# SonyCSLParis/vqcpc-bach

Measured on AMD Instinct MI355X. Metric: encoder-train windows/sec (Bach 4-voice, seq=256), higher is better.
Workload: dtype f32

## Files before the change

vqcpc_bach_amd/csrc/gru.hip:

```cpp
#include "common.h"

namespace vq {

__device__ __forceinline__ float sigmoidf_(float x) { return 1.0f / (1.0f + expf(-x)); }

struct GiTok {
    const int64_t* tokens;
    int L, p, voff, vmax;
};

template <bool TOK>
__device__ __forceinline__ const float* gi_row(const float* gi, const GiTok& tk, int64_t b, int H) {
    if constexpr (TOK) {
        const int tok = min(max((int)tk.tokens[b * tk.L + tk.p], 0), tk.vmax - 1);
        return gi + (int64_t)(tk.voff + tok) * 3 * H;
    } else {
        return gi + b * 3 * H;
    }
}

template <bool TOK>
__global__ __launch_bounds__(256) void gru_cell_fwd_kernel(const float* __restrict__ gi, GiTok tk, const float* __restrict__ gh,
                                                           const float* __restrict__ h_prev, float* __restrict__ h_out,
                                                           float* __restrict__ y_out, int64_t B, int H, uint32_t thr,
                                                           float inv_keep, uint64_t seed, uint64_t idx_base) {
    const int64_t e = (int64_t)blockIdx.x * blockDim.x + threadIdx.x;
    if (e >= B * H) return;
    const int64_t b = e / H;
    const int c = (int)(e - b * H);
    const float* gib = gi_row<TOK>(gi, tk, b, H);
    const float* ghb = gh + b * 3 * H;
    const float r = sigmoidf_(gib[c] + ghb[c]);
    const float u = sigmoidf_(gib[H + c] + ghb[H + c]);
    const float n = tanhf(gib[2 * H + c] + r * ghb[2 * H + c]);
    const float hp = h_prev ? h_prev[e] : 0.0f;
    const float h = (1.0f - u) * n + u * hp;
    h_out[e] = h;
    if (y_out) y_out[e] = h * drop_scale(seed, idx_base + (uint64_t)e, thr, inv_keep);
}

template <bool TOK>
__global__ __launch_bounds__(256) void gru_cell_bwd_kernel(const float* __restrict__ gi, GiTok tk, const float* __restrict__ gh,
                                                           const float* __restrict__ h_prev, const float* __restrict__ d_y,
                                                           const float* __restrict__ d_h, float* __restrict__ d_gi,
                                                           float* __restrict__ d_gh, float* __restrict__ d_hprev, int64_t B,
                                                           int H, uint32_t thr, float inv_keep, uint64_t seed,
                                                           uint64_t idx_base) {
    const int64_t e = (int64_t)blockIdx.x * blockDim.x + threadIdx.x;
    if (e >= B * H) return;
    const int64_t b = e / H;
    const int c = (int)(e - b * H);
    const int64_t o = b * 3 * H + c;
    const float* gib = gi_row<TOK>(gi, tk, b, H) + c;
    const float ghn = gh[o + 2 * H];
    const float r = sigmoidf_(gib[0] + gh[o]);
    const float u = sigmoidf_(gib[H] + gh[o + H]);
    const float n = tanhf(gib[2 * H] + r * ghn);
    const float hp = h_prev ? h_prev[e] : 0.0f;
    float dh = d_h ? d_h[e] : 0.0f;
    if (d_y) dh += d_y[e] * drop_scale(seed, idx_base + (uint64_t)e, thr, inv_keep);
    const float da_n = dh * (1.0f - u) * (1.0f - n * n);
    const float da_u = dh * (hp - n) * u * (1.0f - u);
    const float da_r = da_n * ghn * r * (1.0f - r);
    d_gi[o] = da_r;
    d_gi[o + H] = da_u;
    d_gi[o + 2 * H] = da_n;
    d_gh[o] = da_r;
    d_gh[o + H] = da_u;
    d_gh[o + 2 * H] = da_n * r;
    d_hprev[e] = dh * u;
}

typedef float gru_f16 __attribute__((ext_vector_type(16)));
constexpr int kGruNW = 8;

#define GRU_MFMA4(ACC, AV, BV)                                                     \
    ACC = __builtin_amdgcn_mfma_f32_32x32x2f32(AV.x, BV.x, ACC, 0, 0, 0);           \
    ACC = __builtin_amdgcn_mfma_f32_32x32x2f32(AV.y, BV.y, ACC, 0, 0, 0);           \
    ACC = __builtin_amdgcn_mfma_f32_32x32x2f32(AV.z, BV.z, ACC, 0, 0, 0);           \
    ACC = __builtin_amdgcn_mfma_f32_32x32x2f32(AV.w, BV.w, ACC, 0, 0, 0);

template <bool TOK>
__global__ __launch_bounds__(kGruNW * 64) void gru_step_fwd_kernel(const float* __restrict__ gi, GiTok tk, const float* __restrict__ w_hh,
                                                                   const float* __restrict__ b_hh,
                                                                   const float* __restrict__ h_prev, float* __restrict__ gh,
                                                                   float* __restrict__ h_out, float* __restrict__ y_out,
                                                                   int B, int H, uint32_t thr, float inv_keep, uint64_t seed,
                                                                   uint64_t idx_base) {
    extern __shared__ float gru_red[];
    const int lane = threadIdx.x & 63, wave = threadIdx.x >> 6, g = lane >> 5, l31 = lane & 31;
    const int i = blockIdx.y * 32 + l31, j = blockIdx.x * 32 + l31;
    float e_gi[2][3], e_hp[2];
    int e_row[2];
#pragma unroll
    for (int q = 0; q < 2; ++q) {
        const int r = 2 * wave + q;
        e_row[q] = blockIdx.y * 32 + (r & 3) + 8 * (r >> 2) + 4 * g;
        const int rr = min(e_row[q], B - 1);
        const float* gib = gi_row<TOK>(gi, tk, rr, H) + j;
        e_gi[q][0] = gib[0];
        e_gi[q][1] = gib[H];
        e_gi[q][2] = gib[2 * H];
        e_hp[q] = h_prev ? h_prev[(int64_t)rr * H + j] : 0.0f;
    }
    const float br = b_hh[j], bu = b_hh[H + j], bn = b_hh[2 * H + j];
    gru_f16 acc[3];
#pragma unroll
    for (int q = 0; q < 3; ++q)
#pragma unroll
        for (int r = 0; r < 16; ++r) acc[q][r] = 0.0f;
    if (h_prev != nullptr) {
        const int len = H / (2 * kGruNW);
        const int k0 = (wave * 2 + g) * len;
        const float* ap = h_prev + (int64_t)min(i, B - 1) * H + k0;
        const float* bp = w_hh + (int64_t)j * H + k0;
        int kk = 0;
        for (; kk + 16 <= len; kk += 16) {
            float4 a[4], b[3][4];
#pragma unroll
            for (int v = 0; v < 4; ++v) {
                a[v] = *reinterpret_cast<const float4*>(ap + kk + 4 * v);
#pragma unroll
                for (int q = 0; q < 3; ++q) b[q][v] = *reinterpret_cast<const float4*>(bp + (int64_t)q * H * H + kk + 4 * v);
            }
#pragma unroll
            for (int v = 0; v < 4; ++v) {
                GRU_MFMA4(acc[0], a[v], b[0][v])
                GRU_MFMA4(acc[1], a[v], b[1][v])
                GRU_MFMA4(acc[2], a[v], b[2][v])
            }
        }
        for (; kk < len; kk += 4) {
            const float4 a = *reinterpret_cast<const float4*>(ap + kk);
#pragma unroll
            for (int q = 0; q < 3; ++q) {
                const float4 b = *reinterpret_cast<const float4*>(bp + (int64_t)q * H * H + kk);
                GRU_MFMA4(acc[q], a, b)
            }
        }
#pragma unroll
        for (int q = 0; q < 3; ++q)
#pragma unroll
            for (int r = 0; r < 16; ++r) gru_red[((wave * 3 + q) * 16 + r) * 64 + lane] = acc[q][r];
        __syncthreads();
    }
#pragma unroll
    for (int q = 0; q < 2; ++q) {
        const int r = 2 * wave + q;
        float v3[3] = {0.0f, 0.0f, 0.0f};
        if (h_prev != nullptr) {
#pragma unroll
            for (int w = 0; w < kGruNW; ++w)
#pragma unroll
                for (int t = 0; t < 3; ++t) v3[t] += gru_red[((w * 3 + t) * 16 + r) * 64 + lane];
        }
        if (e_row[q] < B) {
            const float vr = v3[0] + br, vu = v3[1] + bu, vn = v3[2] + bn;
            const int64_t o = (int64_t)e_row[q] * 3 * H + j, e = (int64_t)e_row[q] * H + j;
            gh[o] = vr; gh[o + H] = vu; gh[o + 2 * H] = vn;
            const float rr = sigmoidf_(e_gi[q][0] + vr);
            const float uu = sigmoidf_(e_gi[q][1] + vu);
            const float nn = tanhf(e_gi[q][2] + rr * vn);
            const float hv = (1.0f - uu) * nn + uu * e_hp[q];
            h_out[e] = hv;
            if (y_out) y_out[e] = hv * drop_scale(seed, idx_base + (uint64_t)e, thr, inv_keep);
        }
    }
}

template <bool TOK>
__global__ __launch_bounds__(kGruNW * 64) void gru_step_bwd_kernel(const float* __restrict__ dgh_next,
                                                                   const float* __restrict__ whh_t, float* __restrict__ dhp,
                                                                   const float* __restrict__ gi, GiTok tk, const float* __restrict__ gh,
                                                                   const float* __restrict__ h_prev,
                                                                   const float* __restrict__ d_y, float* __restrict__ d_gi,
                                                                   float* __restrict__ d_gh, int B, int H, uint32_t thr,
                                                                   float inv_keep, uint64_t seed, uint64_t idx_base) {
    extern __shared__ float gru_red[];
    const int lane = threadIdx.x & 63, wave = threadIdx.x >> 6, g = lane >> 5, l31 = lane & 31;
    const int i = blockIdx.y * 32 + l31, j = blockIdx.x * 32 + l31;
    const int K3 = 3 * H;
    float e_gi[2][3], e_gh[2][3], e_hp[2], e_dh[2];
    int e_row[2];
#pragma unroll
    for (int q = 0; q < 2; ++q) {
        const int r = 2 * wave + q;
        e_row[q] = blockIdx.y * 32 + (r & 3) + 8 * (r >> 2) + 4 * g;
        const int rr = min(e_row[q], B - 1);
        const int64_t o = (int64_t)rr * 3 * H + j, e = (int64_t)rr * H + j;
        const float* gib = gi_row<TOK>(gi, tk, rr, H) + j;
#pragma unroll
        for (int t = 0; t < 3; ++t) {
            e_gi[q][t] = gib[(int64_t)t * H];
            e_gh[q][t] = gh[o + (int64_t)t * H];
        }
        e_hp[q] = h_prev ? h_prev[e] : 0.0f;
        e_dh[q] = dhp[e];
        if (d_y) e_dh[q] += d_y[e] * drop_scale(seed, idx_base + (uint64_t)e, thr, inv_keep);
    }
    const int len = K3 / (2 * kGruNW);
    const int k0 = (wave * 2 + g) * len;
    const float* ap = dgh_next + (int64_t)min(i, B - 1) * K3 + k0;
    const float* bp = whh_t + (int64_t)j * K3 + k0;
    gru_f16 acc;
#pragma unroll
    for (int r = 0; r < 16; ++r) acc[r] = 0.0f;
    int kk = 0;
    for (; kk + 32 <= len; kk += 32) {
        float4 a[8], b[8];
#pragma unroll
        for (int v = 0; v < 8; ++v) {
            a[v] = *reinterpret_cast<const float4*>(ap + kk + 4 * v);
            b[v] = *reinterpret_cast<const float4*>(bp + kk + 4 * v);
        }
#pragma unroll
        for (int v = 0; v < 8; ++v) { GRU_MFMA4(acc, a[v], b[v]) }
    }
    for (; kk < len; kk += 4) {
        const float4 a = *reinterpret_cast<const float4*>(ap + kk);
        const float4 b = *reinterpret_cast<const float4*>(bp + kk);
        GRU_MFMA4(acc, a, b)
    }
#pragma unroll
    for (int r = 0; r < 16; ++r) gru_red[(wave * 16 + r) * 64 + lane] = acc[r];
    __syncthreads();
#pragma unroll
    for (int q = 0; q < 2; ++q) {
        const int r = 2 * wave + q;
        float dh = 0.0f;
#pragma unroll
        for (int w = 0; w < kGruNW; ++w) dh += gru_red[(w * 16 + r) * 64 + lane];
        if (e_row[q] < B) {
            const int64_t o = (int64_t)e_row[q] * 3 * H + j, e = (int64_t)e_row[q] * H + j;
            dh += e_dh[q];
            const float ghn = e_gh[q][2];
            const float rr = sigmoidf_(e_gi[q][0] + e_gh[q][0]);
            const float uu = sigmoidf_(e_gi[q][1] + e_gh[q][1]);
            const float nn = tanhf(e_gi[q][2] + rr * ghn);
            const float hp = e_hp[q];
            const float da_n = dh * (1.0f - uu) * (1.0f - nn * nn);
            const float da_u = dh * (hp - nn) * uu * (1.0f - uu);
            const float da_r = da_n * ghn * rr * (1.0f - rr);
            d_gi[o] = da_r; d_gi[o + H] = da_u; d_gi[o + 2 * H] = da_n;
            d_gh[o] = da_r; d_gh[o + H] = da_u; d_gh[o + 2 * H] = da_n * rr;
            dhp[e] = dh * uu;
        }
    }
}
#undef GRU_MFMA4

constexpr int kTokSegU = 16;
constexpr int kTokSegChunkRows = 128;
constexpr int kTokSegMaxChunks = 64;

__global__ __launch_bounds__(256) void gru_tok_segsum_kernel(const float* __restrict__ g, const int64_t* __restrict__ tokens,
                                                             float* __restrict__ ws, int64_t R, int rows_per_chunk, int L, int p,
                                                             int vmax, int C) {
    extern __shared__ __attribute__((aligned(16))) float tok_acc[];
    for (int i = threadIdx.x; i < vmax * 256; i += 256) tok_acc[i] = 0.0f;
    __syncthreads();
    const int ctiles = (C + 255) / 256;
    const int ct = blockIdx.x % ctiles, chunk = blockIdx.x / ctiles;
    const int col = ct * 256 + threadIdx.x;
    const bool cok = col < C;
    const int64_t b0 = (int64_t)chunk * rows_per_chunk;
    const int64_t b1 = min(b0 + rows_per_chunk, R);
    const float* gp = g + (cok ? col : 0);
    float* mine = tok_acc + threadIdx.x;
    for (int64_t b = b0; b < b1; b += kTokSegU) {
        float v[kTokSegU];
        const int64_t trow = min(b + (int)(threadIdx.x & 63) % kTokSegU, b1 - 1);
        const int tokv = min(max((int)tokens[trow * L + p], 0), vmax - 1);
#pragma unroll
        for (int u = 0; u < kTokSegU; ++u) {
            const int64_t row = min(b + u, b1 - 1);
            v[u] = b + u < b1 ? gp[row * C] : 0.0f;
        }
#pragma unroll
        for (int u = 0; u < kTokSegU; ++u) mine[__builtin_amdgcn_readlane(tokv, u) * 256] += v[u];
    }
    if (cok) {
        float* dst = ws + (int64_t)chunk * vmax * C;
        for (int t = 0; t < vmax; ++t) dst[(int64_t)t * C + col] = tok_acc[t * 256 + threadIdx.x];
    }
}

static int tok_segsum_chunks(int64_t R) {
    return (int)std::max<int64_t>(1, std::min<int64_t>(kTokSegMaxChunks, ceil_div(R, kTokSegChunkRows)));
}

static int gi_tok_args(const char* who, const int64_t* tokens, int64_t B, int L, int p, int n_voices, int vmax, GiTok* tk) {
    VQ_REQUIRE(tokens && L >= 1 && p >= 0 && p < L && n_voices >= 1 && vmax >= 1 && B < (1 << 30),
               "%s: bad token arguments (L=%d p=%d n_voices=%d vmax=%d)", who, L, p, n_voices, vmax);
    *tk = GiTok{tokens, L, p, (p % n_voices) * vmax, vmax};
    return VQCPC_OK;
}

}

#include <algorithm>
using namespace vq;

template <bool TOK>
static int cell_fwd_launch(const float* gi, GiTok tk, const float* gh, const float* h_prev, float* h_out, float* y_out, int64_t B,
                           int H, float drop_p, uint64_t seed, uint64_t idx_base, void* stream) {
    VQ_REQUIRE(gi && gh && h_out && B >= 0 && H >= 1, "gru_cell_fwd: bad arguments");
    VQ_REQUIRE(drop_p >= 0.f && drop_p < 1.f, "gru_cell_fwd: bad dropout probability");
    hipLaunchKernelGGL(gru_cell_fwd_kernel<TOK>, dim3((unsigned)ceil_div(B * H, 256)), dim3(256), 0, (hipStream_t)stream, gi, tk, gh,
                       h_prev, h_out, y_out, B, H, drop_threshold(drop_p), 1.0f / (1.0f - drop_p), seed, idx_base);
    VQ_CHECK_LAUNCH("gru_cell_fwd");
    return VQCPC_OK;
}

template <bool TOK>
static int cell_bwd_launch(const float* gi, GiTok tk, const float* gh, const float* h_prev, const float* d_y, const float* d_h,
                           float* d_gi, float* d_gh, float* d_hprev, int64_t B, int H, float drop_p, uint64_t seed,
                           uint64_t idx_base, void* stream) {
    VQ_REQUIRE(gi && gh && d_gi && d_gh && d_hprev && (d_y || d_h) && B >= 0 && H >= 1, "gru_cell_bwd: bad arguments");
    VQ_REQUIRE(drop_p >= 0.f && drop_p < 1.f, "gru_cell_bwd: bad dropout probability");
    hipLaunchKernelGGL(gru_cell_bwd_kernel<TOK>, dim3((unsigned)ceil_div(B * H, 256)), dim3(256), 0, (hipStream_t)stream, gi, tk, gh,
                       h_prev, d_y, d_h, d_gi, d_gh, d_hprev, B, H, drop_threshold(drop_p), 1.0f / (1.0f - drop_p), seed,
                       idx_base);
    VQ_CHECK_LAUNCH("gru_cell_bwd");
    return VQCPC_OK;
}

template <bool TOK>
static int step_fwd_launch(const float* gi, GiTok tk, const float* w_hh, const float* b_hh, const float* h_prev, float* gh,
                           float* h_out, float* y_out, int64_t B, int H, float drop_p, uint64_t seed, uint64_t idx_base,
                           void* stream) {
    VQ_REQUIRE(gi && w_hh && b_hh && gh && h_out, "gru_step_fwd: null pointer");
    VQ_REQUIRE(vqcpc_gru_step_supported(B, H) && B < (1 << 30), "gru_step_fwd: needs H %% 64 == 0 (B=%lld H=%d)", (long long)B, H);
    VQ_REQUIRE(drop_p >= 0.f && drop_p < 1.f, "gru_step_fwd: bad dropout probability");
    VQ_REQUIRE(aligned16(w_hh) && (!h_prev || aligned16(h_prev)), "gru_step_fwd: operands must be 16-byte aligned");
    const size_t lds = (size_t)kGruNW * 3 * 16 * 64 * sizeof(float);
    static bool attr = false;
    if (!attr) {
        (void)hipFuncSetAttribute((const void*)gru_step_fwd_kernel<TOK>, hipFuncAttributeMaxDynamicSharedMemorySize, (int)lds);
        attr = true;
    }
    hipLaunchKernelGGL(gru_step_fwd_kernel<TOK>, dim3(H / 32, (unsigned)ceil_div(B, 32)), dim3(kGruNW * 64), lds, (hipStream_t)stream,
                       gi, tk, w_hh, b_hh, h_prev, gh, h_out, y_out, (int)B, H, drop_threshold(drop_p), 1.0f / (1.0f - drop_p), seed,
                       idx_base);
    VQ_CHECK_LAUNCH("gru_step_fwd");
    return VQCPC_OK;
}

template <bool TOK>
static int step_bwd_launch(const float* dgh_next, const float* whh_t, float* dhp, const float* gi, GiTok tk, const float* gh,
                           const float* h_prev, const float* d_y, float* d_gi, float* d_gh, int64_t B, int H, float drop_p,
                           uint64_t seed, uint64_t idx_base, void* stream) {
    VQ_REQUIRE(dgh_next && whh_t && dhp && gi && gh && d_gi && d_gh, "gru_step_bwd: null pointer");
    VQ_REQUIRE(vqcpc_gru_step_supported(B, H) && B < (1 << 30), "gru_step_bwd: needs H %% 64 == 0 (B=%lld H=%d)", (long long)B, H);
    VQ_REQUIRE(drop_p >= 0.f && drop_p < 1.f, "gru_step_bwd: bad dropout probability");
    VQ_REQUIRE(aligned16(dgh_next) && aligned16(whh_t), "gru_step_bwd: operands must be 16-byte aligned");
    const size_t lds = (size_t)kGruNW * 16 * 64 * sizeof(float);
    hipLaunchKernelGGL(gru_step_bwd_kernel<TOK>, dim3(H / 32, (unsigned)ceil_div(B, 32)), dim3(kGruNW * 64), lds, (hipStream_t)stream,
                       dgh_next, whh_t, dhp, gi, tk, gh, h_prev, d_y, d_gi, d_gh, (int)B, H, drop_threshold(drop_p),
                       1.0f / (1.0f - drop_p), seed, idx_base);
    VQ_CHECK_LAUNCH("gru_step_bwd");
    return VQCPC_OK;
}

extern "C" {

int vqcpc_gru_cell_fwd(const float* gi, const float* gh, const float* h_prev, float* h_out, float* y_out, int64_t B, int H,
                       float drop_p, uint64_t seed, uint64_t idx_base, void* stream) {
    if (B == 0) return VQCPC_OK;
    return cell_fwd_launch<false>(gi, GiTok{}, gh, h_prev, h_out, y_out, B, H, drop_p, seed, idx_base, stream);
}

int vqcpc_gru_cell_bwd(const float* gi, const float* gh, const float* h_prev, const float* d_y, const float* d_h, float* d_gi,
                       float* d_gh, float* d_hprev, int64_t B, int H, float drop_p, uint64_t seed, uint64_t idx_base,
                       void* stream) {
    if (B == 0) return VQCPC_OK;
    return cell_bwd_launch<false>(gi, GiTok{}, gh, h_prev, d_y, d_h, d_gi, d_gh, d_hprev, B, H, drop_p, seed, idx_base, stream);
}

int vqcpc_gru_step_supported(int64_t B, int H) { return (B >= 1 && H >= 64 && H % 64 == 0 && H <= 4096) ? 1 : 0; }

int vqcpc_gru_step_fwd(const float* gi, const float* w_hh, const float* b_hh, const float* h_prev, float* gh, float* h_out,
                       float* y_out, int64_t B, int H, float drop_p, uint64_t seed, uint64_t idx_base, void* stream) {
    if (B == 0) return VQCPC_OK;
    return step_fwd_launch<false>(gi, GiTok{}, w_hh, b_hh, h_prev, gh, h_out, y_out, B, H, drop_p, seed, idx_base, stream);
}

int vqcpc_gru_step_bwd(const float* dgh_next, const float* whh_t, float* dhp, const float* gi, const float* gh,
// ... 74 lines not shown
```

vqcpc_bach_amd/csrc/util.hip:

```cpp
#include <stdarg.h>

#include <algorithm>

#include "common.h"

namespace vq {

static thread_local char g_err[512] = "";

void set_error(const char* fmt, ...) {
    va_list ap;
    va_start(ap, fmt);
    vsnprintf(g_err, sizeof(g_err), fmt, ap);
    va_end(ap);
}

constexpr int kRedCols = 64, kRedGroups = 16;

__global__ __launch_bounds__(kRedCols * kRedGroups) void reduce_splits_kernel(const float* __restrict__ ws,
                                                                              int64_t stride, int nsplit,
                                                                              float* __restrict__ out, int64_t count,
                                                                              const float* __restrict__ ws2, int64_t stride2,
                                                                              float* __restrict__ out2, int64_t count2,
                                                                              int accumulate) {
    __shared__ float part[kRedGroups][kRedCols];
    const int tx = threadIdx.x % kRedCols, ty = threadIdx.x / kRedCols;
    int64_t col = (int64_t)blockIdx.x * kRedCols + tx;
    const int64_t first = (count + kRedCols - 1) / kRedCols * kRedCols;
    if (col >= first) {
        col -= first;
        ws = ws2;
        stride = stride2;
        out = out2;
        count = count2;
    }
    float acc = 0.0f;
    if (col < count) {
        int s = ty;
        for (; s + 3 * kRedGroups < nsplit; s += 4 * kRedGroups) {
            const float a = ws[(int64_t)s * stride + col];
            const float b = ws[(int64_t)(s + kRedGroups) * stride + col];
            const float c = ws[(int64_t)(s + 2 * kRedGroups) * stride + col];
            const float d = ws[(int64_t)(s + 3 * kRedGroups) * stride + col];
            acc = ((acc + a) + b) + (c + d);
        }
        for (; s < nsplit; s += kRedGroups) acc += ws[(int64_t)s * stride + col];
    }
    part[ty][tx] = acc;
    __syncthreads();
    if (ty == 0 && col < count) {
        float tot = accumulate ? out[col] : 0.0f;
#pragma unroll
        for (int g = 0; g < kRedGroups; ++g) tot += part[g][tx];
        out[col] = tot;
    }
}

constexpr int kRedVecThreads = 256;

__global__ __launch_bounds__(kRedVecThreads) void reduce_splits_vec_kernel(const float* __restrict__ ws, int64_t stride,
                                                                          int nsplit, float* __restrict__ out, int64_t count,
                                                                          const float* __restrict__ ws2, int64_t stride2,
                                                                          float* __restrict__ out2, int64_t count2,
                                                                          int accumulate) {
    int64_t q = (int64_t)blockIdx.x * kRedVecThreads + threadIdx.x;
    const int64_t first = (count / 4 + kRedVecThreads - 1) / kRedVecThreads * kRedVecThreads;
    if (q >= first) {
        q -= first;
        ws = ws2;
        stride = stride2;
        out = out2;
        count = count2;
    }
    if (q * 4 >= count) return;
    const float4* p = reinterpret_cast<const float4*>(ws) + q;
    const int64_t st4 = stride / 4;
    float4 acc = make_float4(0.f, 0.f, 0.f, 0.f);
#define RV_ADD(X, Y) make_float4(X.x + Y.x, X.y + Y.y, X.z + Y.z, X.w + Y.w)
    int s = 0;
    for (; s + 7 < nsplit; s += 8) {
        const float4 v0 = p[(s + 0) * st4], v1 = p[(s + 1) * st4], v2 = p[(s + 2) * st4], v3 = p[(s + 3) * st4];
        const float4 v4 = p[(s + 4) * st4], v5 = p[(s + 5) * st4], v6 = p[(s + 6) * st4], v7 = p[(s + 7) * st4];
        const float4 a = RV_ADD(v0, v1), b = RV_ADD(v2, v3), c = RV_ADD(v4, v5), d = RV_ADD(v6, v7);
        const float4 ab = RV_ADD(a, b), cd = RV_ADD(c, d);
        const float4 t = RV_ADD(ab, cd);
        acc = RV_ADD(acc, t);
    }
    for (; s < nsplit; ++s) {
        const float4 v = p[s * st4];
        acc = RV_ADD(acc, v);
    }
    float4* o = reinterpret_cast<float4*>(out) + q;
    if (accumulate) {
        const float4 prev = *o;
        acc = RV_ADD(prev, acc);
    }
#undef RV_ADD
    *o = acc;
}

static bool reduce_vec_ok(const float* ws, int64_t stride, const float* out, int64_t count) {
    return count <= 0 || (count % 4 == 0 && stride % 4 == 0 && aligned16(ws) && aligned16(out));
}

int launch_reduce_splits2(const float* ws, int64_t stride, int nsplit, float* out, int64_t count, const float* ws2,
                          int64_t stride2, float* out2, int64_t count2, int accumulate, hipStream_t stream) {
    if (count <= 0 && count2 <= 0) return VQCPC_OK;
    if (count >= (1 << 16) && nsplit <= 64 && reduce_vec_ok(ws, stride, out, count) &&
        reduce_vec_ok(ws2, stride2, out2, count2)) {
        const int64_t blocks = ceil_div(count / 4, (int64_t)kRedVecThreads) +
                               ceil_div(std::max<int64_t>(count2, 0) / 4, (int64_t)kRedVecThreads);
        hipLaunchKernelGGL(reduce_splits_vec_kernel, dim3((unsigned)blocks), dim3(kRedVecThreads), 0, stream, ws, stride,
                           nsplit, out, count, ws2, stride2, out2, std::max<int64_t>(count2, 0), accumulate);
        VQ_CHECK_LAUNCH("reduce_splits_vec");
        return VQCPC_OK;
    }
    const int64_t blocks = ceil_div(std::max<int64_t>(count, 0), kRedCols) + ceil_div(std::max<int64_t>(count2, 0), kRedCols);
    hipLaunchKernelGGL(reduce_splits_kernel, dim3((unsigned)blocks), dim3(kRedCols * kRedGroups), 0, stream, ws, stride,
                       nsplit, out, std::max<int64_t>(count, 0), ws2, stride2, out2, std::max<int64_t>(count2, 0), accumulate);
    VQ_CHECK_LAUNCH("reduce_splits");
    return VQCPC_OK;
}

constexpr int kRedMany = 32;
struct RedManyArgs {
    const float* ws[kRedMany];
    float* out[kRedMany];
    int stride[kRedMany], nsplit[kRedMany], count[kRedMany];
    int blk_begin[kRedMany + 1];
    int n, accumulate;
};

__global__ __launch_bounds__(kRedCols * kRedGroups) void reduce_many_kernel(const RedManyArgs g) {
    __shared__ float part[kRedGroups][kRedCols];
    const int b = (int)blockIdx.x;
    int p = 0;
    for (int i = 1; i < g.n; ++i) p += (b >= g.blk_begin[i]) ? 1 : 0;
    p = __builtin_amdgcn_readfirstlane(p);
    const float* __restrict__ ws = g.ws[p];
    const int64_t stride = g.stride[p];
    const int nsplit = g.nsplit[p], count = g.count[p];
    const int tx = threadIdx.x % kRedCols, ty = threadIdx.x / kRedCols;
    const int col = (b - g.blk_begin[p]) * kRedCols + tx;
    float acc = 0.0f;
    if (col < count) {
        int s = ty;
        for (; s + 3 * kRedGroups < nsplit; s += 4 * kRedGroups) {
            const float a = ws[(int64_t)s * stride + col];
            const float b2 = ws[(int64_t)(s + kRedGroups) * stride + col];
            const float c = ws[(int64_t)(s + 2 * kRedGroups) * stride + col];
            const float d = ws[(int64_t)(s + 3 * kRedGroups) * stride + col];
            acc = ((acc + a) + b2) + (c + d);
        }
        for (; s < nsplit; s += kRedGroups) acc += ws[(int64_t)s * stride + col];
    }
    part[ty][tx] = acc;
    __syncthreads();
    if (ty == 0 && col < count) {
        float* out = g.out[p];
        float tot = g.accumulate ? out[col] : 0.0f;
#pragma unroll
        for (int q = 0; q < kRedGroups; ++q) tot += part[q][tx];
        out[col] = tot;
    }
}

__global__ __launch_bounds__(kRedVecThreads) void reduce_many_vec_kernel(const RedManyArgs g) {
    const int b = (int)blockIdx.x;
    int p = 0;
    for (int i = 1; i < g.n; ++i) p += (b >= g.blk_begin[i]) ? 1 : 0;
    p = __builtin_amdgcn_readfirstlane(p);
    const int64_t q = (int64_t)(b - g.blk_begin[p]) * kRedVecThreads + threadIdx.x;
    if (q * 4 >= g.count[p]) return;
    const float4* ptr = reinterpret_cast<const float4*>(g.ws[p]) + q;
    const int64_t st4 = g.stride[p] / 4;
    const int nsplit = g.nsplit[p];
    float4 acc = make_float4(0.f, 0.f, 0.f, 0.f);
#define RV_ADD(X, Y) make_float4(X.x + Y.x, X.y + Y.y, X.z + Y.z, X.w + Y.w)
    int s = 0;
    for (; s + 7 < nsplit; s += 8) {
        const float4 v0 = ptr[(s + 0) * st4], v1 = ptr[(s + 1) * st4], v2 = ptr[(s + 2) * st4], v3 = ptr[(s + 3) * st4];
        const float4 v4 = ptr[(s + 4) * st4], v5 = ptr[(s + 5) * st4], v6 = ptr[(s + 6) * st4], v7 = ptr[(s + 7) * st4];
        const float4 a = RV_ADD(v0, v1), bb = RV_ADD(v2, v3), c = RV_ADD(v4, v5), d = RV_ADD(v6, v7);
        const float4 ab = RV_ADD(a, bb), cd = RV_ADD(c, d);
        const float4 t = RV_ADD(ab, cd);
        acc = RV_ADD(acc, t);
    }
    for (; s < nsplit; ++s) {
        const float4 v = ptr[s * st4];
        acc = RV_ADD(acc, v);
    }
    float4* o = reinterpret_cast<float4*>(g.out[p]) + q;
    if (g.accumulate) {
        const float4 prev = *o;
        acc = RV_ADD(prev, acc);
    }
#undef RV_ADD
    *o = acc;
}

int launch_reduce_splits(const float* ws, int64_t stride, int nsplit, float* out, int64_t count, int accumulate,
                         hipStream_t stream) {
    return launch_reduce_splits2(ws, stride, nsplit, out, count, nullptr, 0, nullptr, 0, accumulate, stream);
}

__global__ __launch_bounds__(256) void dropout_mask_kernel(float* mask, int64_t n, uint32_t thr, uint64_t seed) {
    int64_t i = (int64_t)blockIdx.x * blockDim.x + threadIdx.x;
    const int64_t step = (int64_t)gridDim.x * blockDim.x;
    for (; i < n; i += step) mask[i] = (thr == 0 || rng_u24(seed, (uint64_t)i) >= thr) ? 1.0f : 0.0f;
}

__global__ __launch_bounds__(256) void transpose_kernel(const float* __restrict__ in, float* __restrict__ out, int R,
                                                        int C) {
    __shared__ float tile[32][33];
    const int tx = threadIdx.x & 31, ty = threadIdx.x >> 5;
    const int c0 = blockIdx.x * 32, r0 = blockIdx.y * 32;
#pragma unroll
    for (int k = 0; k < 4; ++k) {
        int r = r0 + ty + k * 8, c = c0 + tx;
        if (r < R && c < C) tile[ty + k * 8][tx] = in[(int64_t)r * C + c];
    }
    __syncthreads();
#pragma unroll
    for (int k = 0; k < 4; ++k) {
        int c = c0 + ty + k * 8, r = r0 + tx;
        if (r < R && c < C) out[(int64_t)c * R + r] = tile[tx][ty + k * 8];
    }
}

__global__ __launch_bounds__(256) void transpose_many_kernel(const float* __restrict__ base_in, float* __restrict__ base_out,
                                                             const int64_t* __restrict__ desc, int n) {
    __shared__ float tile[32][33];
    int lo = 0, hi = n - 1;
    const int64_t t = blockIdx.x;
    while (lo < hi) {
        const int mid = (lo + hi + 1) >> 1;
        if (desc[4 * mid + 3] <= t) lo = mid; else hi = mid - 1;
    }
    const int64_t off = desc[4 * lo];
    const int R = (int)desc[4 * lo + 1], C = (int)desc[4 * lo + 2];
    const int local = (int)(t - desc[4 * lo + 3]), tiles_c = (C + 31) / 32;
    const float* in = base_in + off;
    float* out = base_out + off;
    const int tx = threadIdx.x & 31, ty = threadIdx.x >> 5;
    const int c0 = (local % tiles_c) * 32, r0 = (local / tiles_c) * 32;
#pragma unroll
    for (int k = 0; k < 4; ++k) {
        const int r = r0 + ty + k * 8, c = c0 + tx;
        if (r < R && c < C) tile[ty + k * 8][tx] = in[(int64_t)r * C + c];
    }
    __syncthreads();
#pragma unroll
    for (int k = 0; k < 4; ++k) {
        const int c = c0 + ty + k * 8, r = r0 + tx;
        if (r < R && c < C) out[(int64_t)c * R + r] = tile[tx][ty + k * 8];
    }
}

__device__ __forceinline__ float selu_f(float h, float s) {
    const double alpha = 1.6732632423543772848170429916717, scale = 1.0507009873554804934193349852946;
    const double x = (double)h * (double)s;
    return (float)(scale * (x > 0.0 ? x : alpha * expm1(x)));
}
__device__ __forceinline__ float selu_grad(float x) {
    const float alpha = 1.6732632423543772848170429916717f, scale = 1.0507009873554804934193349852946f;
    return scale * (x > 0.0f ? 1.0f : alpha * __expf(x));
}

__global__ __launch_bounds__(256) void dropout_selu_fwd_kernel(const float* __restrict__ h, float* __restrict__ out,
                                                               int64_t n, uint32_t thr, float inv_keep, uint64_t seed) {
    int64_t i = (int64_t)blockIdx.x * blockDim.x + threadIdx.x;
    const int64_t step = (int64_t)gridDim.x * blockDim.x;
// ... 69 lines not shown
        v[i] = vi;
        g[i] = gi;
        p[i] -= lr_over_bc1 * (mi / (sqrtf(vi) * inv_sqrt_bc2 + eps));
    }
}


static SaltAddrFn g_salt_fns[32];
static int g_salt_nfn = 0;
void register_rng_salt(SaltAddrFn fn) {
    if (g_salt_nfn < 32) g_salt_fns[g_salt_nfn++] = fn;
}
struct SaltAddrs {
    uint64_t* p[32];
    int n;
};
static SaltAddrs salt_addrs() {
    static SaltAddrs a = [] {
        SaltAddrs r{};
        for (int i = 0; i < g_salt_nfn; ++i) {
            uint64_t* q = g_salt_fns[i]();
            if (q) r.p[r.n++] = q;
        }
        return r;
    }();
    return a;
}
__device__ __forceinline__ uint64_t splitmix64(uint64_t x) {
    x += 0x9E3779B97F4A7C15ull;
    x = (x ^ (x >> 30)) * 0xBF58476D1CE4E5B9ull;
    x = (x ^ (x >> 27)) * 0x94D049BB133111EBull;
    return x ^ (x >> 31);
}
__global__ void rng_salt_set_kernel(SaltAddrs a, uint64_t value) {
    if (threadIdx.x < a.n) *a.p[threadIdx.x] = value;
}
__global__ void rng_salt_advance_kernel(SaltAddrs a, uint64_t* counter, uint64_t base) {
    __shared__ uint64_t salt;
    if (threadIdx.x == 0) {
        const uint64_t c = counter[0] + 1;
        counter[0] = c;
        const uint64_t v = splitmix64(base ^ c);
        salt = v ? v : 1;
    }
    __syncthreads();
    if (threadIdx.x < a.n) *a.p[threadIdx.x] = salt;
}
__global__ void rng_salt_from_counter_kernel(SaltAddrs a, const uint64_t* counter, uint64_t base) {
    const uint64_t v = splitmix64(base ^ counter[0]);
    if (threadIdx.x < a.n) *a.p[threadIdx.x] = v ? v : 1;
}

__global__ __launch_bounds__(256) void adam_dev_kernel(float* __restrict__ p, float* __restrict__ g, float* __restrict__ m,
                                                       float* __restrict__ v, int64_t n, const float* __restrict__ lr_dev,
                                                       float beta1, float beta2, float eps,
                                                       const uint64_t* __restrict__ step_dev, float grad_scale,
                                                       float max_norm, const double* __restrict__ sumsq) {
    __shared__ float sh[2];
    if (threadIdx.x == 0) {
        const double t = (double)step_dev[0];
        const double bc1 = 1.0 - pow((double)beta1, t), bc2 = 1.0 - pow((double)beta2, t);
        sh[0] = (float)((double)lr_dev[0] / bc1);
        sh[1] = (float)(1.0 / sqrt(bc2));
    }
    __syncthreads();
    const float lr_over_bc1 = sh[0], inv_sqrt_bc2 = sh[1];
    float coef = grad_scale;
    if (sumsq != nullptr) {
        const float total = (float)sqrt(sumsq[0]);
        coef *= fminf(1.0f, max_norm / (total + 1e-6f));
    }
    for (int64_t i = (int64_t)blockIdx.x * 256 + threadIdx.x; i < n; i += (int64_t)gridDim.x * 256) {
        const float gi = g[i] * coef;
        const float mi = beta1 * m[i] + (1.0f - beta1) * gi;
        const float vi = beta2 * v[i] + (1.0f - beta2) * gi * gi;
        m[i] = mi;
        v[i] = vi;
        g[i] = gi;
        p[i] -= lr_over_bc1 * (mi / (sqrtf(vi) * inv_sqrt_bc2 + eps));
    }
}

constexpr int kWeightAverageBlocks = 2048;

__device__ __forceinline__ float weight_average_one(float a, float p, float w) {
#pragma clang fp contract(off)
    const float diff = p - a;
    const float step = w * diff;
    return a + step;
}

__global__ __launch_bounds__(256) void weight_average_kernel(float* __restrict__ avg, const float* __restrict__ p, int64_t n,
                                                             int64_t head, int64_t n4, float decay, uint64_t u,
                                                             const uint64_t* __restrict__ step_dev, uint64_t t0) {
#pragma clang fp contract(off)
    if (step_dev != nullptr) {
        const uint64_t t = step_dev[0];
        if (t <= t0) return;
        u = t - t0;
    }
    const float ratio = (float)(1 + u) / (float)(10 + u);
    const float d = fminf(decay, ratio);
    const float w = 1.0f - d;
    const int64_t stride = (int64_t)gridDim.x * 256;
    const int64_t first = (int64_t)blockIdx.x * 256 + threadIdx.x;
    float4* a4 = reinterpret_cast<float4*>(avg + head);
    const float4* p4 = reinterpret_cast<const float4*>(p + head);
    for (int64_t i = first; i < n4; i += stride) {
        float4 a = a4[i];
        const float4 q = p4[i];
        a.x = weight_average_one(a.x, q.x, w);
        a.y = weight_average_one(a.y, q.y, w);
        a.z = weight_average_one(a.z, q.z, w);
        a.w = weight_average_one(a.w, q.w, w);
        a4[i] = a;
    }
    const int64_t rest = n - 4 * n4;
    for (int64_t j = first; j < rest; j += stride) {
        const int64_t i = j < head ? j : j + 4 * n4;
        avg[i] = weight_average_one(avg[i], p[i], w);
    }
}

struct TokenLimits {
    int v[16];
};
__global__ __launch_bounds__(256) void check_tokens_kernel(const int64_t* __restrict__ in, int64_t n, int nv,
                                                           TokenLimits lim, int64_t* __restrict__ out,
                                                           int* __restrict__ flag) {
    bool bad = false;
    for (int64_t i = (int64_t)blockIdx.x * 256 + threadIdx.x; i < n; i += (int64_t)gridDim.x * 256) {
        const int64_t t = in[i];
        const int64_t hi = lim.v[(int)(i % nv)] - 1;
        const int64_t c = t < 0 ? 0 : (t > hi ? hi : t);
        bad |= c != t;
        out[i] = c;
    }
    if (__any(bad) && (threadIdx.x & 63) == 0) atomicOr(flag, 1);
}

struct Acc8 {
    float* dst[8];
    const float* src[8];
    int n[8];
};
__global__ __launch_bounds__(256) void accumulate8_kernel(Acc8 a) {
    const int t = blockIdx.y;
    float* d = a.dst[t];
    const float* s = a.src[t];
    const int n = a.n[t];
    for (int i = blockIdx.x * 256 + threadIdx.x; i < n; i += gridDim.x * 256) d[i] += s[i];
}

constexpr int kCountThreads = 1024;
constexpr int64_t kCountMaxSpace = 1 << 20;

__global__ __launch_bounds__(kCountThreads) void count_distinct_codes_kernel(const int64_t* __restrict__ idx_a, int64_t rows_a,
                                                                            const int64_t* __restrict__ idx_b, int64_t rows_b,
                                                                            int ncb, int K, int words, float* __restrict__ out) {
    extern __shared__ uint32_t code_bits[];
    __shared__ int wave_tot[kCountThreads / 64];
    for (int i = threadIdx.x; i < words; i += kCountThreads) code_bits[i] = 0u;
    __syncthreads();
    for (int64_t i = threadIdx.x; i < rows_a + rows_b; i += kCountThreads) {
        const int64_t* row = i < rows_a ? idx_a + i * ncb : idx_b + (i - rows_a) * ncb;
        int64_t code = 0, mul = 1;
        for (int c = 0; c < ncb; ++c) {
            code += row[c] * mul;
            mul *= K;
        }
        if (code >= 0 && code < (int64_t)words * 32) atomicOr(&code_bits[code >> 5], 1u << (code & 31));
    }
    __syncthreads();
    int cnt = 0;
    for (int i = threadIdx.x; i < words; i += kCountThreads) cnt += __popc(code_bits[i]);
#pragma unroll
    for (int o = 32; o > 0; o >>= 1) cnt += __shfl_xor(cnt, o, 64);
    if ((threadIdx.x & 63) == 0) wave_tot[threadIdx.x >> 6] = cnt;
    __syncthreads();
    if (threadIdx.x == 0) {
        int tot = 0;
        for (int w = 0; w < kCountThreads / 64; ++w) tot += wave_tot[w];
        out[0] = (float)tot;
    }
}

}

using namespace vq;

extern "C" {

int vqcpc_abi_version(void) { return VQCPC_ABI_VERSION; }
const char* vqcpc_last_error(void) { return vq::g_err; }
int vqcpc_clear_runtime_error(void) { return (int)hipGetLastError(); }

int vqcpc_dropout_mask(float* mask, int64_t n, float p, uint64_t seed, void* stream) {
    if (n == 0) return VQCPC_OK;
    VQ_REQUIRE(mask != nullptr && n >= 0 && p >= 0.f && p < 1.f, "dropout_mask: bad arguments");
    int blocks = (int)std::min<int64_t>(ceil_div(n, 256), 4096);
    hipLaunchKernelGGL(dropout_mask_kernel, dim3(blocks), dim3(256), 0, (hipStream_t)stream, mask, n, drop_threshold(p),
                       seed);
    VQ_CHECK_LAUNCH("dropout_mask");
    return VQCPC_OK;
}

int vqcpc_transpose(const float* in, float* out, int R, int C, void* stream) {
    VQ_REQUIRE(in && out && R > 0 && C > 0, "transpose: bad arguments");
    hipLaunchKernelGGL(transpose_kernel, dim3(ceil_div(C, 32), ceil_div(R, 32)), dim3(256), 0, (hipStream_t)stream, in,
                       out, R, C);
    VQ_CHECK_LAUNCH("transpose");
    return VQCPC_OK;
}

int vqcpc_transpose_many(const float* base_in, float* base_out, const int64_t* desc, int n, int64_t total_tiles,
                         void* stream) {
    if (n == 0) return VQCPC_OK;
    VQ_REQUIRE(base_in && base_out && desc && n > 0 && total_tiles > 0 && total_tiles < (1ll << 31) && base_in != base_out,
               "transpose_many: bad arguments");
    hipLaunchKernelGGL(transpose_many_kernel, dim3((unsigned)total_tiles), dim3(256), 0, (hipStream_t)stream, base_in, base_out,
                       desc, n);
    VQ_CHECK_LAUNCH("transpose_many");
    return VQCPC_OK;
}

int vqcpc_dropout_selu_fwd(const float* h, float* out, int64_t n, float drop_p, uint64_t seed, void* stream) {
    if (n == 0) return VQCPC_OK;
    VQ_REQUIRE(h && out && n >= 0 && drop_p >= 0.f && drop_p < 1.f, "dropout_selu_fwd: bad arguments");
    int blocks = (int)std::min<int64_t>(ceil_div(n, 256), 4096);
    hipLaunchKernelGGL(dropout_selu_fwd_kernel, dim3(blocks), dim3(256), 0, (hipStream_t)stream, h, out, n,
                       drop_threshold(drop_p), 1.0f / (1.0f - drop_p), seed);
    VQ_CHECK_LAUNCH("dropout_selu_fwd");
    return VQCPC_OK;
}

int vqcpc_dropout_selu_bwd(const float* h, const float* g_out, float* g_h, int64_t n, float drop_p, uint64_t seed,
                           void* stream) {
    if (n == 0) return VQCPC_OK;
    VQ_REQUIRE(h && g_out && g_h && n >= 0 && drop_p >= 0.f && drop_p < 1.f, "dropout_selu_bwd: bad arguments");
    int blocks = (int)std::min<int64_t>(ceil_div(n, 256), 4096);
    hipLaunchKernelGGL(dropout_selu_bwd_kernel, dim3(blocks), dim3(256), 0, (hipStream_t)stream, h, g_out, g_h, n,
                       drop_threshold(drop_p), 1.0f / (1.0f - drop_p), seed);
    VQ_CHECK_LAUNCH("dropout_selu_bwd");
    return VQCPC_OK;
}

int64_t vqcpc_sumsq_workspace(int64_t n) {
    (void)n;
    return (int64_t)kSumsqBlocks * sizeof(double);
}

int vqcpc_sumsq(const float* g, int64_t n, float grad_scale, double* out, void* workspace, int64_t workspace_bytes,
                void* stream) {
    VQ_REQUIRE(g && out && workspace && n > 0, "sumsq: bad arguments");
    VQ_REQUIRE(aligned16(g), "sumsq: g must be 16-byte aligned");
    if (workspace_bytes < vqcpc_sumsq_workspace(n)) {
        set_error("sumsq: workspace too small");
        return VQCPC_EWORKSPACE;
    }
    int blocks = (int)std::min<int64_t>(ceil_div(n / 4 + 1, 256), kSumsqBlocks);
    hipLaunchKernelGGL(sumsq_stage1, dim3(blocks), dim3(256), 0, (hipStream_t)stream, g, n, grad_scale,
                       (double*)workspace);
    VQ_CHECK_LAUNCH("sumsq_stage1");
    hipLaunchKernelGGL(sumsq_stage2, dim3(1), dim3(256), 0, (hipStream_t)stream, (const double*)workspace, blocks, out);
    VQ_CHECK_LAUNCH("sumsq_stage2");
    return VQCPC_OK;
}

int vqcpc_adam_step(float* p, float* g, float* m, float* v, int64_t n, float lr, float beta1, float beta2, float eps,
                    int step, float grad_scale, float max_norm, const double* sumsq, void* stream) {
    VQ_REQUIRE(p && g && m && v && n > 0 && step >= 1, "adam_step: bad arguments");
    const double bc1 = 1.0 - pow((double)beta1, (double)step);
    const double bc2 = 1.0 - pow((double)beta2, (double)step);
    int blocks = (int)std::min<int64_t>(ceil_div(n, 256), 4096);
    hipLaunchKernelGGL(adam_kernel, dim3(blocks), dim3(256), 0, (hipStream_t)stream, p, g, m, v, n, (float)(lr / bc1),
                       beta1, beta2, eps, (float)(1.0 / sqrt(bc2)), grad_scale, max_norm, sumsq);
    VQ_CHECK_LAUNCH("adam_step");
    return VQCPC_OK;
}

int vqcpc_check_tokens(const int64_t* tokens, int64_t n, int n_voices, const int32_t* limits, int64_t* clamped, int32_t* flag,
                       void* stream) {
    if (n == 0) return VQCPC_OK;
    VQ_REQUIRE(tokens && limits && clamped && flag && n > 0 && n_voices >= 1 && n_voices <= 16,
               "check_tokens: bad arguments (n_voices <= 16)");
    TokenLimits lim;
    for (int i = 0; i < 16; ++i) lim.v[i] = i < n_voices ? limits[i] : 1;
    for (int i = 0; i < n_voices; ++i) VQ_REQUIRE(lim.v[i] >= 1, "check_tokens: empty vocabulary for voice %d", i);
    int blocks = (int)std::min<int64_t>(ceil_div(n, 256), 2048);
    hipLaunchKernelGGL(check_tokens_kernel, dim3(blocks), dim3(256), 0, (hipStream_t)stream, tokens, n, n_voices, lim,
                       clamped, flag);
    VQ_CHECK_LAUNCH("check_tokens");
    return VQCPC_OK;
}

int vqcpc_rng_salt_set(uint64_t value, void* stream) {
    const SaltAddrs a = salt_addrs();
    hipLaunchKernelGGL(rng_salt_set_kernel, dim3(1), dim3(64), 0, (hipStream_t)stream, a, value);
    VQ_CHECK_LAUNCH("rng_salt_set");
    return VQCPC_OK;
}

int vqcpc_rng_salt_advance(uint64_t* counter, uint64_t base, void* stream) {
    VQ_REQUIRE(counter != nullptr, "rng_salt_advance: null counter");
    const SaltAddrs a = salt_addrs();
    hipLaunchKernelGGL(rng_salt_advance_kernel, dim3(1), dim3(64), 0, (hipStream_t)stream, a, counter, base);
    VQ_CHECK_LAUNCH("rng_salt_advance");
    return VQCPC_OK;
}

int vqcpc_rng_salt_from_counter(const uint64_t* counter, uint64_t base, void* stream) {
    VQ_REQUIRE(counter != nullptr, "rng_salt_from_counter: null counter");
    const SaltAddrs a = salt_addrs();
    hipLaunchKernelGGL(rng_salt_from_counter_kernel, dim3(1), dim3(64), 0, (hipStream_t)stream, a, counter, base);
    VQ_CHECK_LAUNCH("rng_salt_from_counter");
    return VQCPC_OK;
}

int vqcpc_adam_step_dev(float* p, float* g, float* m, float* v, int64_t n, const float* lr_dev, float beta1, float beta2,
                        float eps, const uint64_t* step_dev, float grad_scale, float max_norm, const double* sumsq,
                        void* stream) {
    VQ_REQUIRE(p && g && m && v && lr_dev && step_dev && n > 0, "adam_step_dev: bad arguments");
    int blocks = (int)std::min<int64_t>(ceil_div(n, 256), 4096);
    hipLaunchKernelGGL(adam_dev_kernel, dim3(blocks), dim3(256), 0, (hipStream_t)stream, p, g, m, v, n, lr_dev, beta1, beta2,
// ... 160 lines not shown
```

Measured before the change: 11890.

## Tune GRU backward scheduling, adapt split-reduce width, batch distinct-code counting

Result: no change. 11970 (median of 6 runs) (+0.7%).

```diff
diff --git a/vqcpc_bach_amd/csrc/gru.hip b/vqcpc_bach_amd/csrc/gru.hip
--- a/vqcpc_bach_amd/csrc/gru.hip
+++ b/vqcpc_bach_amd/csrc/gru.hip
@@ -169,7 +169,7 @@
 }
 
 template <bool TOK>
-__global__ __launch_bounds__(kGruNW * 64) void gru_step_bwd_kernel(const float* __restrict__ dgh_next,
+__global__ __launch_bounds__(kGruNW * 64) __attribute__((amdgpu_waves_per_eu(2, 2))) void gru_step_bwd_kernel(const float* __restrict__ dgh_next,
                                                                    const float* __restrict__ whh_t, float* __restrict__ dhp,
                                                                    const float* __restrict__ gi, GiTok tk, const float* __restrict__ gh,
                                                                    const float* __restrict__ h_prev,
@@ -180,7 +180,7 @@
     const int lane = threadIdx.x & 63, wave = threadIdx.x >> 6, g = lane >> 5, l31 = lane & 31;
     const int i = blockIdx.y * 32 + l31, j = blockIdx.x * 32 + l31;
     const int K3 = 3 * H;
-    float e_gi[2][3], e_gh[2][3], e_hp[2], e_dh[2];
+    float e_gi[2][3], e_gh[2][3], e_hp[2], e_dh[2], e_dy[2];
     int e_row[2];
 #pragma unroll
     for (int q = 0; q < 2; ++q) {
@@ -196,7 +196,7 @@
         }
         e_hp[q] = h_prev ? h_prev[e] : 0.0f;
         e_dh[q] = dhp[e];
-        if (d_y) e_dh[q] += d_y[e] * drop_scale(seed, idx_base + (uint64_t)e, thr, inv_keep);
+        e_dy[q] = d_y ? d_y[e] : 0.0f;
     }
     const int len = K3 / (2 * kGruNW);
     const int k0 = (wave * 2 + g) * len;
@@ -213,6 +213,7 @@
             a[v] = *reinterpret_cast<const float4*>(ap + kk + 4 * v);
             b[v] = *reinterpret_cast<const float4*>(bp + kk + 4 * v);
         }
+        __builtin_amdgcn_sched_barrier(0);
 #pragma unroll
         for (int v = 0; v < 8; ++v) { GRU_MFMA4(acc, a[v], b[v]) }
     }
@@ -232,7 +233,9 @@
         for (int w = 0; w < kGruNW; ++w) dh += gru_red[(w * 16 + r) * 64 + lane];
         if (e_row[q] < B) {
             const int64_t o = (int64_t)e_row[q] * 3 * H + j, e = (int64_t)e_row[q] * H + j;
-            dh += e_dh[q];
+            float dhe = e_dh[q];
+            if (d_y) dhe += e_dy[q] * drop_scale(seed, idx_base + (uint64_t)e, thr, inv_keep);
+            dh += dhe;
             const float ghn = e_gh[q][2];
             const float rr = sigmoidf_(e_gi[q][0] + e_gh[q][0]);
             const float uu = sigmoidf_(e_gi[q][1] + e_gh[q][1]);
diff --git a/vqcpc_bach_amd/csrc/util.hip b/vqcpc_bach_amd/csrc/util.hip
--- a/vqcpc_bach_amd/csrc/util.hip
+++ b/vqcpc_bach_amd/csrc/util.hip
@@ -1,6 +1,7 @@
 #include <stdarg.h>
 
 #include <algorithm>
+#include <type_traits>
 
 #include "common.h"
 
@@ -16,17 +17,19 @@
 }
 
 constexpr int kRedCols = 64, kRedGroups = 16;
-
-__global__ __launch_bounds__(kRedCols * kRedGroups) void reduce_splits_kernel(const float* __restrict__ ws,
-                                                                              int64_t stride, int nsplit,
-                                                                              float* __restrict__ out, int64_t count,
-                                                                              const float* __restrict__ ws2, int64_t stride2,
-                                                                              float* __restrict__ out2, int64_t count2,
-                                                                              int accumulate) {
-    __shared__ float part[kRedGroups][kRedCols];
-    const int tx = threadIdx.x % kRedCols, ty = threadIdx.x / kRedCols;
-    int64_t col = (int64_t)blockIdx.x * kRedCols + tx;
-    const int64_t first = (count + kRedCols - 1) / kRedCols * kRedCols;
+constexpr int kRedShortBlocks = 128, kRedShortSplits = 64;
+
+template <int COLS>
+__global__ __launch_bounds__(COLS * kRedGroups) void reduce_splits_kernel(const float* __restrict__ ws,
+                                                                          int64_t stride, int nsplit,
+                                                                          float* __restrict__ out, int64_t count,
+                                                                          const float* __restrict__ ws2, int64_t stride2,
+                                                                          float* __restrict__ out2, int64_t count2,
+                                                                          int accumulate) {
+    __shared__ float part[kRedGroups][COLS];
+    const int tx = threadIdx.x % COLS, ty = threadIdx.x / COLS;
+    int64_t col = (int64_t)blockIdx.x * COLS + tx;
+    const int64_t first = (count + COLS - 1) / COLS * COLS;
     if (col >= first) {
         col -= first;
         ws = ws2;
@@ -37,6 +40,13 @@
     float acc = 0.0f;
     if (col < count) {
         int s = ty;
+        for (; s + 15 * kRedGroups < nsplit; s += 16 * kRedGroups) {
+            float v[16];
+#pragma unroll
+            for (int u = 0; u < 16; ++u) v[u] = ws[(int64_t)(s + u * kRedGroups) * stride + col];
+#pragma unroll
+            for (int u = 0; u < 16; u += 4) acc = ((acc + v[u]) + v[u + 1]) + (v[u + 2] + v[u + 3]);
+        }
         for (; s + 3 * kRedGroups < nsplit; s += 4 * kRedGroups) {
             const float a = ws[(int64_t)s * stride + col];
             const float b = ws[(int64_t)(s + kRedGroups) * stride + col];
@@ -115,9 +125,17 @@
         VQ_CHECK_LAUNCH("reduce_splits_vec");
         return VQCPC_OK;
     }
-    const int64_t blocks = ceil_div(std::max<int64_t>(count, 0), kRedCols) + ceil_div(std::max<int64_t>(count2, 0), kRedCols);
-    hipLaunchKernelGGL(reduce_splits_kernel, dim3((unsigned)blocks), dim3(kRedCols * kRedGroups), 0, stream, ws, stride,
-                       nsplit, out, std::max<int64_t>(count, 0), ws2, stride2, out2, std::max<int64_t>(count2, 0), accumulate);
+    const int64_t c1 = std::max<int64_t>(count, 0), c2 = std::max<int64_t>(count2, 0);
+    const auto launch = [&](auto cols) {
+        constexpr int COLS = decltype(cols)::value;
+        const int64_t blocks = ceil_div(c1, (int64_t)COLS) + ceil_div(c2, (int64_t)COLS);
+        hipLaunchKernelGGL(reduce_splits_kernel<COLS>, dim3((unsigned)blocks), dim3(COLS * kRedGroups), 0, stream, ws, stride,
+                           nsplit, out, c1, ws2, stride2, out2, c2, accumulate);
+    };
+    const auto blocks_at = [&](int cols) { return ceil_div(c1, (int64_t)cols) + ceil_div(c2, (int64_t)cols); };
+    if (nsplit < kRedShortSplits || blocks_at(64) >= kRedShortBlocks) launch(std::integral_constant<int, 64>{});
+    else if (blocks_at(32) >= kRedShortBlocks) launch(std::integral_constant<int, 32>{});
+    else launch(std::integral_constant<int, 16>{});
     VQ_CHECK_LAUNCH("reduce_splits");
     return VQCPC_OK;
 }
@@ -493,7 +511,7 @@
     for (int i = blockIdx.x * 256 + threadIdx.x; i < n; i += gridDim.x * 256) d[i] += s[i];
 }
 
-constexpr int kCountThreads = 1024;
+constexpr int kCountThreads = 1024, kCountBatch = 8;
 constexpr int64_t kCountMaxSpace = 1 << 20;
 
 __global__ __launch_bounds__(kCountThreads) void count_distinct_codes_kernel(const int64_t* __restrict__ idx_a, int64_t rows_a,
@@ -503,14 +521,39 @@
     __shared__ int wave_tot[kCountThreads / 64];
     for (int i = threadIdx.x; i < words; i += kCountThreads) code_bits[i] = 0u;
     __syncthreads();
-    for (int64_t i = threadIdx.x; i < rows_a + rows_b; i += kCountThreads) {
-        const int64_t* row = i < rows_a ? idx_a + i * ncb : idx_b + (i - rows_a) * ncb;
-        int64_t code = 0, mul = 1;
-        for (int c = 0; c < ncb; ++c) {
-            code += row[c] * mul;
-            mul *= K;
-        }
-        if (code >= 0 && code < (int64_t)words * 32) atomicOr(&code_bits[code >> 5], 1u << (code & 31));
+    const int64_t rows = rows_a + rows_b, space = (int64_t)words * 32;
+    const auto mark = [&](int64_t code) {
+        if (code < 0 || code >= space) return;
+        const uint32_t bit = 1u << (code & 31);
+        if (!(__atomic_load_n(&code_bits[code >> 5], __ATOMIC_RELAXED) & bit)) atomicOr(&code_bits[code >> 5], bit);
+    };
+    for (int64_t i0 = threadIdx.x; i0 < rows; i0 += (int64_t)kCountBatch * kCountThreads) {
+        int64_t code[kCountBatch];
+#pragma unroll
+        for (int u = 0; u < kCountBatch; ++u) {
+            const int64_t i = i0 + (int64_t)u * kCountThreads;
+            code[u] = -1;
+            if (i < rows) {
+                const int64_t* row = i < rows_a ? idx_a + i * ncb : idx_b + (i - rows_a) * ncb;
+                code[u] = row[0];
+            }
+        }
+        if (ncb > 1) {
+            int64_t mul = K;
+            for (int c = 1; c < ncb; ++c, mul *= K) {
+                int64_t digit[kCountBatch];
+#pragma unroll
+                for (int u = 0; u < kCountBatch; ++u) {
+                    const int64_t i = i0 + (int64_t)u * kCountThreads;
+                    digit[u] = 0;
+                    if (i < rows) digit[u] = (i < rows_a ? idx_a + i * ncb : idx_b + (i - rows_a) * ncb)[c];
+                }
+#pragma unroll
+                for (int u = 0; u < kCountBatch; ++u) code[u] += digit[u] * mul;
+            }
+        }
+#pragma unroll
+        for (int u = 0; u < kCountBatch; ++u) mark(code[u]);
     }
     __syncthreads();
     int cnt = 0;
```
